# rjzhb/VectorSearch-RBAC

Hardware: AMD Instinct MI355X
Metric: QPS at recall@100, SIFT10M filtered-kNN (role RBAC), 1/2/4/8 MI355X (higher is better)
Workload: dtype int8 planes -> i32 (exact: bit-identical to the fp32 distances of vector.c)

## Files before the change

### vectorsearch-rbac_amd/csrc/vsr_device.h

```cpp
#pragma once
#include <hip/hip_runtime.h>
#include <stdint.h>
#include "vsr_bounds.h"

namespace vsr {

using f32x4 = __attribute__((ext_vector_type(4))) float;
using u32x4 = __attribute__((ext_vector_type(4))) uint32_t;
using i32x4 = __attribute__((ext_vector_type(4))) int;
using bf16x8 = __attribute__((ext_vector_type(8))) __bf16;
using f16x8 = __attribute__((ext_vector_type(8))) _Float16;

#ifdef __HIPCC__
template <class T> using gptr = const __attribute__((address_space(1))) T*;
template <class T> __device__ __forceinline__ gptr<T> as_global(const T* p) { return (gptr<T>) p; }
template <class T> __device__ __forceinline__ T lds_peek(const T* p)
{
    return *(const volatile __attribute__((address_space(3))) T*) p;
}
__device__ __forceinline__ uint2 load_tile(gptr<uint2> tiles, uint32_t t)
{
    const uint64_t v = ((gptr<uint64_t>) tiles)[t];
    return make_uint2((uint32_t) v, (uint32_t) (v >> 32));
}
// ... 16 lines not shown
    const uint64_t* bitmap;
    uint32_t        n_tiles;
    uint32_t        q_begin;
    uint32_t        q_count;
    uint32_t        block_begin;
    uint32_t        n_blocks;
    uint32_t        partial_begin;
};

struct FusedTail {
    uint32_t        enable;
    uint32_t        fan;
    ScanGroup       group;
    uint32_t*       done;
    const int64_t*  block_ids;
    const int32_t*  doc_ids;
    const int64_t*  orig_rows;
    int64_t*        out_block;
    int32_t*        out_doc;
    int64_t*        out_row;
    float*          out_dist;
    uint64_t*       out_keys;
    int32_t*        out_count;
    int32_t*        out_flag;
    int32_t*        flag_total;
    uint32_t        row_offset;
    int             metric;
    uint64_t*       dbg;
};

#ifndef VSR_MW_DENSE
#define VSR_MW_DENSE 1
#endif

struct ScanParams {
    const float4*    rows;
    const float*     norm2;
    uint32_t         n_rows;
    uint32_t         stride4;
    const float*     queries;
    const float*     q_norm2;
    const ScanGroup* groups;
    uint32_t         n_groups;
    const uint32_t*  q_slots;
    uint64_t*        partial;
    uint32_t         kp;
    uint32_t         k;
    uint32_t         cap;
    uint32_t         qmax;
    uint64_t*        cand;
    uint32_t         rw;
    const uint64_t*  tau_init;
    uint32_t         sample_stride;
    const uint2*     block_map;
    const uint4*     scr;
    const uint4*     q_scr;
    uint32_t         pstride4;
    const uint4*     scr_c;
    const uint4*     q_scr_c;
    uint32_t         cstride4;
    uint32_t         plane_ho;
    uint64_t*        qcand;
    uint32_t*        qcnt;
    uint32_t         capq;
    const uint32_t*  rank;
    const uint64_t*  ones;
    uint32_t*        err;
    uint32_t         epi;
    uint32_t         k2i;
    uint32_t         dense;
    FusedTail        fused;
    const uint64_t*  sp_off;
    const uint2*     sp_tab;
    uint32_t         sp_slots;
    const double*    sp_qtot;
};

struct SelectQuery {
    uint32_t ids_begin;
    uint32_t n_lists;
    uint32_t out_slot;
    uint32_t dst_list;
    uint32_t allowed;
    uint32_t pad;
};

constexpr uint32_t SEL_FINAL = 0xFFFFFFFFu;
constexpr uint32_t SEL_SEED = 0xFFFFFFFEu;

struct SelectParams {
    uint64_t*          tau_out;
    int32_t*           out_flags;
    int32_t*           flagged_total;
    int                seeded;
    uint64_t*          partial;
    const uint32_t*    list_ids;
    const SelectQuery* queries;
    uint32_t           kp;
    uint32_t           k;
    uint32_t           cap;
    int                metric;
    uint32_t           row_offset;
    const int64_t*     block_ids;
// ... 243 lines not shown
```

### vectorsearch-rbac_amd/csrc/vsr_mfmaw.h

```cpp
#pragma once
#include <type_traits>
#include "vsr_device.h"
#include "vsr_scan.h"
#include "vsr_topk.h"
#include "vsr_mfma.h"
#include "vsr_i8s.h"
#include "vsr_i8r.h"

namespace vsr {

constexpr int MW_THREADS = 256;
constexpr int MW_WAVES = 4;
constexpr int MW_S = 16;
constexpr int MW_ROWS = 64;
constexpr int MW_NQ = MF_NQ * MW_WAVES;
constexpr int MW_RING = 8;

#ifndef VSR_MW_DEPTH1
#define VSR_MW_DEPTH1 1
#endif
#ifndef VSR_MW_OCC1
#define VSR_MW_OCC1 3
#endif
#ifndef VSR_ABLATE
// ... 11 lines not shown
#define VSR_MW_OCC8 4
#endif
#ifndef VSR_MW_OCCL
#define VSR_MW_OCCL 2
#endif
constexpr int mw_occ(int nch, int pl = 0, bool sample = false)
{
    (void) sample;
    return pl == 2 ? VSR_MW_OCC8 : nch == 1 ? VSR_MW_OCC1 : nch == 0 ? VSR_MW_OCCL : 2;
}

__device__ __forceinline__ void lds_barrier()
{
    asm volatile("s_waitcnt lgkmcnt(0)\n\ts_barrier" ::: "memory");
}

template <int METRIC, int NCH, bool SAMPLE, int PL, int DEPTH, int EPI = 0, int NGT = 1, bool DENSE = false>
__global__ __launch_bounds__(MW_THREADS, mw_occ(NCH, PL, SAMPLE)) void mfma_wide_kernel(const ScanParams p)
{
    constexpr bool HO = PL == 1, I8 = PL == 2;
    constexpr bool LONG = NCH == 0;
    constexpr int NCHR = LONG ? 1 : NCH;
    constexpr int SR = I8 ? 8 : MW_S;
    constexpr int NU = I8 ? 2 : 4;
    static_assert(!I8 || (NCH == 1 && METRIC == M_L2), "int8 planes: one stage (d <= 128), L2 only");
    static_assert(!LONG || DEPTH == 1, "long rows: one stage ahead");
    static_assert(!DENSE || (I8 && !SAMPLE), "dense rows: the int8 main launch only");
    static_assert(DEPTH >= 1 && DEPTH <= 4 && DEPTH + 2 <= MW_RING, "row-mapping ring too short");
    extern __shared__ __align__(16) unsigned char smem[];
    const int tid = threadIdx.x;
    const int lane = tid & 63;
    const int wave = __builtin_amdgcn_readfirstlane(tid >> 6);

    uint32_t lo = 0, mapped_block = 0;
    if (p.block_map) {
        const uint2 m = p.block_map[blockIdx.x];
        if (m.x == 0xFFFFFFFFu) return;
        lo = m.x;
        mapped_block = m.y;
    } else {
        uint32_t hi = p.n_groups;
        while (hi - lo > 1) {
            const uint32_t mid = (lo + hi) >> 1;
            if (p.groups[mid].block_begin <= blockIdx.x) lo = mid; else hi = mid;
        }
    }
    const ScanGroup grp = p.groups[lo];
    const uint32_t local_block = p.block_map ? mapped_block : blockIdx.x - grp.block_begin;
    const auto g_tiles = as_global(grp.tiles);
    const auto g_bitmap = as_global(grp.bitmap);
    const auto g_norm2 = as_global(p.norm2);
    const auto g_ones = as_global(p.ones);
    const auto g_rank = as_global(p.rank);

    const uint32_t pstride4 = p.pstride4;
    const uint32_t q_count = grp.q_count;
    const bool sample_fine = SAMPLE && (grp.partial_begin & 1u);

    uint4*    stage = reinterpret_cast<uint4*>(smem);
    unsigned char* after = smem + 2 * MW_ROWS * SR * 16;
    int32_t*  rowidx = reinterpret_cast<int32_t*>(after);
    float*    rownorm = reinterpret_cast<float*>(after + MW_RING * 64 * 4);
    unsigned char* pend = after + MW_RING * 64 * 8;
    uint32_t* pend_v = reinterpret_cast<uint32_t*>(pend) + (size_t) wave * MW_PEND;
    uint32_t* pend_r = reinterpret_cast<uint32_t*>(pend + 4 * MW_PEND * 4) + (size_t) wave * MW_PEND;
    uint32_t* pend_c = reinterpret_cast<uint32_t*>(pend + 8 * MW_PEND * 4) + (size_t) wave * MW_PEND;
    constexpr bool ITEST = I8 && EPI == 1 && !SAMPLE && METRIC == M_L2;
    int32_t* rowthr = reinterpret_cast<int32_t*>(pend + 12 * MW_PEND * 4);

    const uint32_t ngt = (q_count + MF_NQ - 1) / MF_NQ;
    const uint32_t rsplit = ngt == 1 ? 4u : ngt == 2 ? 2u : 1u;
    const uint32_t g0 = (uint32_t) wave / rsplit;
    const uint32_t sub0 = ((uint32_t) wave % rsplit) * (4u / rsplit);
    const bool gact = g0 < ngt;

    const int li = lane & 15;
    const int kq = lane >> 4;
    const int jq = li;
    constexpr int NBLK = I8 ? 2 : HO ? 4 : 2;
    bf16x8 bh[NCHR][NBLK], bm[NCHR][NBLK];
    const uint4* my_qsrc = nullptr;
    i32x4 b8[NBLK];
    const uint32_t my_qi = g0 * MF_NQ + (uint32_t) jq < (uint32_t) MW_NQ ? g0 * MF_NQ + (uint32_t) jq : 0u;
    float my_qn;
    uint32_t my_slot;
    uint64_t my_tau;
    {
        const uint32_t slot = p.q_slots[grp.q_begin + (my_qi < q_count ? my_qi : 0)];
        my_slot = slot;
        my_tau = p.tau_init ? p.tau_init[slot] : KEY_EMPTY;
        my_qn = p.q_norm2[slot];
        const uint4* qsrc = p.q_scr + (size_t) slot * (HO ? 2 * pstride4 : pstride4);
        my_qsrc = qsrc;
        if constexpr (I8) {
#pragma unroll
            for (int blk = 0; blk < NBLK; ++blk) b8[blk] = __builtin_bit_cast(i32x4, qsrc[blk * 4 + kq]);
        } else {
#pragma unroll
            for (int s = 0; s < NCHR; ++s)
#pragma unroll
                for (int blk = 0; blk < NBLK; ++blk) {
                    bh[s][blk] = __builtin_bit_cast(bf16x8, qsrc[s * (HO ? 32 : 16) + blk * 4 + kq]);
                    bm[s][blk] = __builtin_bit_cast(bf16x8, qsrc[s * (HO ? 32 : 16) + (HO ? 16 : 8) + blk * 4 + kq]);
                }
        }
    }

    const uint32_t rw = p.rw, tps = MW_ROWS / rw;
    const uint32_t t0 = (uint32_t) (((uint64_t) grp.n_tiles * local_block) / grp.n_blocks);
    const uint32_t t1 = (uint32_t) (((uint64_t) grp.n_tiles * (local_block + 1)) / grp.n_blocks);
    const uint32_t n_super = (t1 - t0 + tps - 1) / tps;
    const uint32_t ss = p.sample_stride;
    const uint32_t n_it = (VSR_ABLATE & 16) ? 0u : (n_super + ss - 1) / ss;
    const bool qok = my_qi < q_count;
    const bool open = my_tau == KEY_EMPTY;
    const float tau_lim = open ? __builtin_inff() : mono_to_float((uint32_t) (my_tau >> 32));
    const int32_t c0 = !qok ? -0x40000000 : open ? 0x3FFFFFFF : (((int32_t) tau_lim - (int32_t) my_qn) + 1) >> 1;
    constexpr int NG = NGT;
    static_assert(NG == 1 || LONG, "two query groups per wave: long rows only");
    const uint32_t g1 = (uint32_t) wave + 4u;
    const bool gact2 = NG == 2 && rsplit == 1u && g1 < ngt;
    const uint32_t my_qi2 = g1 * MF_NQ + (uint32_t) jq;
    const bool qok2 = gact2 && my_qi2 < q_count;
    uint32_t my_slot2 = my_slot;
    float my_qn2 = 0.0f, tau_lim2 = -__builtin_inff();
    const uint4* my_qsrc2 = nullptr;
    bf16x8 bh2[NBLK], bm2[NBLK];
    if constexpr (NG == 2) {
        my_slot2 = p.q_slots[grp.q_begin + (qok2 ? my_qi2 : 0u)];
        const uint64_t t2 = p.tau_init ? p.tau_init[my_slot2] : KEY_EMPTY;
        tau_lim2 = t2 == KEY_EMPTY ? __builtin_inff() : mono_to_float((uint32_t) (t2 >> 32));
        my_qn2 = p.q_norm2[my_slot2];
        my_qsrc2 = p.q_scr + (size_t) my_slot2 * (HO ? 2 * pstride4 : pstride4);
#pragma unroll
        for (int blk = 0; blk < NBLK; ++blk) {
            bh2[blk] = __builtin_bit_cast(bf16x8, my_qsrc2[blk * 4 + kq]);
            bm2[blk] = __builtin_bit_cast(bf16x8, my_qsrc2[(HO ? 16 : 8) + blk * 4 + kq]);
        }
    }
    const uint32_t col_slot = lane < MF_NQ ? my_slot : my_slot2;

    const uint32_t tile_last = grp.n_tiles - 1u;
    auto fetch_desc = [&](uint32_t it_) -> uint2 {
        const uint32_t t = t0 + it_ * ss * tps + (uint32_t) lane / rw;
        const bool ok = it_ < n_it && t < t1;
        const uint2 d = load_tile(g_tiles, t < tile_last ? t : tile_last);
        return make_uint2(ok ? d.x : 0u, ok ? d.y : 0u);
    };
    int32_t  pend_row[DEPTH];
    uint64_t pend_bw[DEPTH];
    float    pend_nrm[DEPTH];
    uint2    dsc_a[DEPTH];
#pragma unroll
    for (int j = 0; j < DEPTH; ++j) {
        pend_row[j] = -1;
        pend_bw[j] = ~0ull;
        pend_nrm[j] = 0.0f;
        dsc_a[j] = make_uint2(0u, 0u);
    }
    bool bad_row = false;
    uint32_t row_lo = 0, row_hi = 0;
    if constexpr (DENSE) {
        const uint2 da = load_tile(g_tiles, t0 < tile_last ? t0 : tile_last);
        const uint2 db = load_tile(g_tiles, t1 > t0 && t1 - 1u < tile_last ? t1 - 1u : tile_last);
        row_lo = (uint32_t) __builtin_amdgcn_readfirstlane((int) da.x);
        row_hi = t1 > t0 ? (uint32_t) __builtin_amdgcn_readfirstlane((int) (db.x + db.y)) : row_lo;
        bad_row = row_hi > p.n_rows || row_hi < row_lo;
        row_hi = bad_row ? row_lo : row_hi;
    }
    auto start_dense = [&](uint32_t it_, int32_t& row, uint64_t& bw, float& nrm) {
        const uint32_t rr = row_lo + it_ * (uint32_t) MW_ROWS + (uint32_t) lane;
        const bool ok = it_ < n_it && rr < row_hi;
        row = ok ? (int32_t) rr : -1;
        bw = ~0ull;
        nrm = g_norm2[ok ? rr : 0u];
    };
    auto start_rows = [&](uint2 d, int32_t& row, uint64_t& bw, float& nrm) {
        const uint32_t r = (uint32_t) lane % rw;
        const uint32_t rr = d.x + r;
        const bool ok = r < d.y && rr < p.n_rows;
        bad_row |= r < d.y && rr >= p.n_rows;
        const uint32_t rc = ok ? rr : 0u;
        row = ok ? (int32_t) rr : -1;
        bw = *(g_bitmap ? g_bitmap + (rc >> 6) : g_ones);
        nrm = g_norm2[rc];
    };
    auto finish_rows = [&](uint32_t it_, int32_t row, uint64_t bw, float nrm) {
        if (row >= 0 && !((bw >> ((uint32_t) row & 63u)) & 1ull)) row = -1;
        if (wave == 0) {
            rowidx[(it_ % MW_RING) * 64 + lane] = row;
            rownorm[(it_ % MW_RING) * 64 + lane] = row >= 0 ? nrm : __builtin_nanf("");
            if constexpr (ITEST) rowthr[(it_ % MW_RING) * 64 + lane] = row >= 0 ? ((int32_t) nrm) >> 1 : 0x7FFFFFFF;
        }
    };
    if constexpr (DENSE) {
#pragma unroll
        for (int j = 0; j < DEPTH; ++j) {
            int32_t r0;
            uint64_t b0;
            float n0;
            start_dense((uint32_t) j, r0, b0, n0);
            finish_rows((uint32_t) j, r0, b0, n0);
            start_dense((uint32_t) (DEPTH + j), pend_row[j], pend_bw[j], pend_nrm[j]);
        }
    } else {
        uint2 d[2 * DEPTH];
#pragma unroll
        for (int j = 0; j < 2 * DEPTH; ++j) d[j] = fetch_desc((uint32_t) j);
#pragma unroll
        for (int j = 0; j < DEPTH; ++j) dsc_a[j] = fetch_desc((uint32_t) (2 * DEPTH + j));
#pragma unroll
        for (int j = 0; j < DEPTH; ++j) {
            int32_t r0;
            uint64_t b0;
            float n0;
            start_rows(d[j], r0, b0, n0);
            finish_rows((uint32_t) j, r0, b0, n0);
            start_rows(d[DEPTH + j], pend_row[j], pend_bw[j], pend_nrm[j]);
        }
    }
    __syncthreads();

    const int lrow = I8 ? tid >> 3 : tid >> 4, lchunk = I8 ? tid & 7 : tid & 15;
    constexpr int LROWS = I8 ? 32 : 16;
    uint4 X[DEPTH][NCHR][NU];
    const uint32_t last_row = p.n_rows - 1u;
    auto issue = [&](auto dc, auto sc, uint32_t it_) {
        constexpr int D = decltype(dc)::value;
        constexpr int S = decltype(sc)::value;
        const uint32_t chunk = (uint32_t) (S * SR + lchunk);
        const int32_t* ridx = rowidx + (it_ % MW_RING) * 64;
#pragma unroll
        for (int u = 0; u < NU; ++u) {
            uint32_t rc;
            if constexpr (DENSE) {
                const uint32_t rr = row_lo + it_ * (uint32_t) MW_ROWS + (uint32_t) (u * LROWS + lrow);
                rc = it_ < n_it && rr < row_hi ? rr : 0u;
            } else {
                const int32_t r = ridx[u * LROWS + lrow];
                rc = (uint32_t) (r < 0 ? 0 : r);
            }
            if ((VSR_ABLATE & 8) && it_ > 0) continue;
            const u32x4 v = *reinterpret_cast<const u32x4*>(p.scr + (size_t) (rc < last_row ? rc : last_row) * pstride4 + chunk);
            X[D][S][u] = make_uint4(v[0], v[1], v[2], v[3]);
        }
    };
    const uint32_t nch_rt = LONG ? pstride4 / (uint32_t) SR : (uint32_t) NCH;
    auto issue_rt = [&](uint32_t it_, uint32_t s_) {
        const uint32_t chunk = s_ * (uint32_t) SR + (uint32_t) lchunk;
        const int32_t* ridx = rowidx + (it_ % MW_RING) * 64;
#pragma unroll
        for (int u = 0; u < NU; ++u) {
            const int32_t r = ridx[u * LROWS + lrow];
            const uint32_t rc = (uint32_t) (r < 0 ? 0 : r);
            const u32x4 v = *reinterpret_cast<const u32x4*>(p.scr + (size_t) (rc < last_row ? rc : last_row) * pstride4 + chunk);
            X[0][0][u] = make_uint4(v[0], v[1], v[2], v[3]);
        }
    };
    auto load_b = [&](uint32_t s_, bf16x8 (&h)[NBLK], bf16x8 (&m)[NBLK]) {
#pragma unroll
        for (int blk = 0; blk < NBLK; ++blk) {
            h[blk] = __builtin_bit_cast(bf16x8, my_qsrc[s_ * (HO ? 32u : 16u) + (uint32_t) (blk * 4 + kq)]);
            m[blk] = __builtin_bit_cast(bf16x8, my_qsrc[s_ * (HO ? 32u : 16u) + (HO ? 16u : 8u) + (uint32_t) (blk * 4 + kq)]);
        }
    };
    auto issue_tile = [&](auto dc, uint32_t it_) {
        if constexpr (LONG) {
            issue_rt(it_, 0u);
            return;
        }
        issue(dc, std::integral_constant<int, 0>{}, it_);
        if constexpr (NCH > 1) issue(dc, std::integral_constant<int, 1>{}, it_);
        if constexpr (NCH > 2) issue(dc, std::integral_constant<int, 2>{}, it_);
    };
    const uint32_t n_pad = (n_it + DEPTH - 1) / DEPTH * DEPTH;
    issue_tile(std::integral_constant<int, 0>{}, 0);
    if constexpr (DEPTH > 1) issue_tile(std::integral_constant<int, 1>{}, 1);
    if constexpr (DEPTH > 2) issue_tile(std::integral_constant<int, 2>{}, 2);
    if constexpr (DEPTH > 3) issue_tile(std::integral_constant<int, 3>{}, 3);

    uint32_t p_head = 0, p_tail = 0, f_n = 0;
    constexpr int FL_R = 2;
    uint32_t f_rank[FL_R];
    uint32_t f_base = 0;
#pragma unroll
    for (int r = 0; r < FL_R; ++r) f_rank[r] = 0;
    auto flush_issue = [&]() __attribute__((always_inline)) {
        const uint32_t have = p_tail - p_head;
        f_n = have < 64u * FL_R ? have : 64u * FL_R;
        uint32_t col[FL_R];
#pragma unroll
        for (int r = 0; r < FL_R; ++r) {
            const uint32_t e = (uint32_t) (r * 64 + lane);
            col[r] = e < f_n ? pend_c[(p_head + e) % MW_PEND] : 0xFFu;
        }
        uint32_t mine = 0;
#pragma unroll
        for (int c = 0; c < MF_NQ * NG; ++c) {
            uint32_t before = 0;
#pragma unroll
            for (int r = 0; r < FL_R; ++r) {
                const uint64_t m = __ballot(col[r] == (uint32_t) c);
                if (col[r] == (uint32_t) c)
                    f_rank[r] = before + __builtin_amdgcn_mbcnt_hi((uint32_t) (m >> 32), __builtin_amdgcn_mbcnt_lo((uint32_t) m, 0u));
                before += (uint32_t) __popcll(m);
            }
            if (lane == c) mine = before;
        }
        if (lane < MF_NQ * NG && mine) f_base = atomicAdd(p.qcnt + col_slot, mine);
    };
    auto flush_store = [&]() __attribute__((always_inline)) {
#pragma unroll
        for (int r = 0; r < FL_R; ++r) {
            const uint32_t e = (uint32_t) (r * 64 + lane);
            const uint32_t idx = (p_head + e) % MW_PEND;
            const uint32_t c = e < f_n ? pend_c[idx] : 0u;
            const uint32_t base = (uint32_t) __shfl((int) f_base, (int) c);
            const uint32_t slot = (uint32_t) __shfl((int) col_slot, (int) c);
            if (e < f_n) {
                const uint32_t row = pend_r[idx];
                const uint32_t at = base + f_rank[r];
                if (at < p.capq)
                    p.qcand[(size_t) slot * p.capq + at] = ((uint64_t) pend_v[idx] << 32) | (g_rank ? g_rank[row] : row);
            }
        }
        p_head += f_n;
        f_n = 0;
    };
    auto park_mask = [&](uint64_t act, bool has, uint32_t key_hi, uint32_t row, uint32_t col = 0xFFFFFFFFu, uint32_t slot_ = 0u)
                         __attribute__((always_inline)) {
        if (col == 0xFFFFFFFFu) {
            col = (uint32_t) jq;
            slot_ = my_slot;
        }
        const uint32_t room = MW_PEND - (p_tail - p_head);
        const uint32_t rank = __builtin_amdgcn_mbcnt_hi((uint32_t) (act >> 32), __builtin_amdgcn_mbcnt_lo((uint32_t) act, 0u));
        if (has) {
            if (rank < room) {
                const uint32_t at = (p_tail + rank) % MW_PEND;
                pend_v[at] = key_hi;
                pend_r[at] = row;
                pend_c[at] = col;
            } else {
                const uint32_t ga = atomicAdd(p.qcnt + slot_, 1u);
                if (ga < p.capq) p.qcand[(size_t) slot_ * p.capq + ga] = ((uint64_t) key_hi << 32) | (g_rank ? g_rank[row] : row);
            }
        }
        const uint32_t n_act = (uint32_t) __popcll(act);
        p_tail += n_act < room ? n_act : room;
    };
    auto park = [&](bool has, uint32_t key_hi, uint32_t row, uint32_t col = 0xFFFFFFFFu, uint32_t slot_ = 0u)
                    __attribute__((always_inline)) {
        park_mask(__ballot(has), has, key_hi, row, col, slot_);
    };

    auto run = [&](auto nsc) {
// ... 378 lines not shown
```

### vectorsearch-rbac_amd/csrc/vsr_plan.h

```cpp
#pragma once
#include "vsr_runtime.h"

namespace vsr {

constexpr uint32_t SEL_FANIN = 64;

struct PlanScalars {
    uint32_t n_blocks = 0;
    int      qi = 1;
    bool     mq = false;
    bool     k2 = false;
    bool     k2w = false;
    bool     int8 = false;
    bool     class_view = false;
    bool     k2g = false;
    bool     sparse_global = false;
    uint32_t keep = 0;
    uint32_t rerank_base = 0;
    uint32_t n_scan_lists = 0;
    uint32_t qmax = 1;
    bool     k2i_sample = false;
    bool     k2r_sample = false;
    uint32_t n_blocks_s = 0;
    uint32_t n_partial_s = 0;
    uint32_t n_partial = 0;
    bool     sel_wave = false;
    uint32_t n_launch = 0;
    int64_t  scan_rows = 0;
    int64_t  scan_bytes = 0;
    float    kp_frac = 0;
    uint32_t sample_stride = 1;
    int64_t  scan_pairs = 0;
    int64_t  unique_rows = 0;
};

struct Plan : PlanScalars {
    std::vector<uint32_t>    q_slots;
    std::vector<ScanGroup>   groups;
    std::vector<uint32_t>    list_ids;
    std::vector<SelectQuery> sel1;
    std::vector<SelectQuery> selq;
    std::vector<ScanGroup>   groups_s;
    std::vector<SelectQuery> seedq;
    std::vector<uint2>       block_map;

    void reset()
    {
        static_cast<PlanScalars&>(*this) = PlanScalars{};
        q_slots.clear(); groups.clear(); list_ids.clear(); sel1.clear(); selq.clear(); groups_s.clear(); seedq.clear(); block_map.clear();
    }
};

bool make_plan(const vsr_ctx* ctx, const vsr_corpus* c, int nq, int k, int metric, bool allow_screening, bool allow_wide,
               bool allow_gemm, const vsr_filter* const* filters, Plan& plan);

inline double seed_lambda(uint32_t kp, double frac) { return (double) kp * frac; }
uint32_t seed_rank(uint32_t kp, double frac);

std::string scan_kernel_name(const Plan& plan, const vsr_corpus* c, int metric, bool k2i = false);

}
```

### vectorsearch-rbac_amd/csrc/vsr_plan.hip

```cpp
#include "vsr_plan.h"

#include <cmath>
#include <cstdio>

namespace {

struct PlanIn {
    const vsr_ctx*           ctx;
    const vsr_corpus*        c;
    int                      nq, k, metric;
    const vsr_filter* const* filters;
    const vsr_filter* filter(uint32_t q) const { return filters ? filters[q] : nullptr; }
};

struct PassItem { const vsr_filter* part; uint32_t slot; };
struct Pass {
    const vsr_filter* f; uint32_t q_off, q_count; int64_t rows; uint32_t n_tiles; int64_t cost;
    const uint2* vtiles;
};

constexpr uint32_t XCDS = 8;

struct PlanScratch {
    std::vector<PassItem> raw, items;
    std::vector<uint32_t> gid;
    std::vector<uint32_t> gend;
    std::vector<const vsr_filter*> gpart;
    std::vector<Pass>     passes;
    std::vector<uint32_t> loff, lcur, lids, lids_s, lcnt_s, level2;
    std::vector<double>   gdens_s;
    std::vector<double>   est;
    std::vector<uint2>    lane[XCDS];
};

struct Width {
    bool     mq_ok, k2_ok, k2w_ok, k2g, i8wide;
    int      wq;
    int      qmax;
    uint32_t keep, keep_c;
};

struct LaunchSize {
    int64_t  budget;
    int64_t  total_cost;
    uint32_t seed_div;
};

int64_t group_items(const PlanIn& in, PlanScratch& s)
{
    static std::atomic<uint64_t> g_epoch{0};
    const uint64_t epoch = g_epoch.fetch_add(1, std::memory_order_relaxed) + 1;
    s.raw.clear(); s.gid.clear(); s.gend.clear(); s.gpart.clear();
    const bool decompose = in.nq >= 32 && !in.ctx->no_classes;
    uint32_t null_group = 0xFFFFFFFFu;
    auto add = [&](const vsr_filter* f, uint32_t q) {
        uint32_t g;
        if (!f) {
            if (null_group == 0xFFFFFFFFu) {
                null_group = (uint32_t) s.gpart.size();
                s.gpart.push_back(nullptr);
                s.gend.push_back(0);
            }
            g = null_group;
        } else {
            if (f->plan_epoch != epoch) {
// ... 135 lines not shown
    bool any = false;
    for (const Pass& p : passes) {
        const vsr_filter* f = p.f;
        if (f && f->scanned_rows == 0) continue;
        if (!f || f->view_class < 0 || (size_t) f->view_class >= v->rows.size() || f->mode != VSR_FILTER_RANGES || f->d_bitmap ||
            f->allowed_rows != f->scanned_rows || f->scanned_rows != (int64_t) v->rows[(size_t) f->view_class])
            return false;
        any = true;
    }
    if (!any) return false;
    for (Pass& p : passes) {
        if (!p.f || p.f->scanned_rows == 0) continue;
        const size_t cls = (size_t) p.f->view_class;
        p.vtiles = v->d_tiles + v->start[cls] / 16;
        p.n_tiles = (v->rows[cls] + 15) / 16;
    }
    return true;
}

LaunchSize size_launch(const PlanIn& in, const Plan& plan, const std::vector<Pass>& passes)
{
    const vsr_ctx* ctx = in.ctx;
    int64_t total_rows = 0;
    LaunchSize ls{};
    for (auto& p : passes) {
        total_rows += std::max<int64_t>(p.rows, 1);
        ls.total_cost += p.cost;
    }
    const int64_t cus = ctx->prop.multiProcessorCount;
    ls.budget = ctx->block_budget > 0 ? ctx->block_budget : in.nq == 1 ? 2 * cus : 4 * cus;
    ls.seed_div = ctx->seed_block_div;
    if (ctx->block_budget <= 0 && plan.qi == 4) {
        const int64_t want = plan.k2g ? std::min<int64_t>(total_rows / 2048, 3 * cus)
                           : plan.k2w ? std::min<int64_t>(total_rows / 4096, 12 * cus) : std::min<int64_t>(total_rows / 13000, 16 * cus);
        if (want > ls.budget) {
            ls.budget = want;
            ls.seed_div = std::max<uint32_t>(ls.seed_div, (uint32_t) (ls.budget / (2 * cus)));
        }
    }
    if (plan.k2w) {
        const int64_t slots = (plan.k2g ? 1 : plan.int8 ? 4 : 3) * cus * ctx->sample_rounds;
        ls.seed_div = (uint32_t) std::max<int64_t>(1, (ls.budget + slots - 1) / slots);
    }
    return ls;
}

void emit_groups(const PlanIn& in, bool i8wide, const LaunchSize& ls, PlanScratch& s, Plan& plan)
{
    const vsr_ctx* ctx = in.ctx;
    const vsr_corpus* c = in.c;
    s.gdens_s.clear();
    s.loff.assign((size_t) in.nq + 1, 0);
    for (auto& p : s.passes) {
        if (p.n_tiles == 0 || p.rows == 0) continue;
        int64_t nb = (int64_t) (((__int128) p.cost * ls.budget + ls.total_cost - 1) / ls.total_cost);
        const int64_t min_rows = p.q_count > 1 ? std::max<int64_t>(ctx->min_rows_per_block, ctx->min_shared_rows) : ctx->min_rows_per_block;
        nb = std::min<int64_t>(nb, std::max<int64_t>(1, p.rows / min_rows));
        nb = std::min<int64_t>(nb, std::max<uint32_t>(1, p.n_tiles));
        nb = std::max<int64_t>(nb, 1);
        ScanGroup g;
        g.tiles = p.vtiles ? p.vtiles : p.f ? p.f->d_tiles : plan.k2w ? c->d_all_tiles : nullptr;
        g.bitmap = p.f ? p.f->d_bitmap : nullptr;
        g.n_tiles = p.n_tiles;
        g.q_begin = p.q_off;
        g.q_count = p.q_count;
        g.block_begin = plan.n_blocks;
        g.n_blocks = (uint32_t) nb;
        g.partial_begin = plan.n_partial;
        plan.groups.push_back(g);
        const double dens = p.f && p.f->scanned_rows > 0 ? (double) p.f->allowed_rows / (double) p.f->scanned_rows : 1.0;
        ScanGroup gs = g;
        gs.n_blocks = (uint32_t) std::max<int64_t>(1, nb / ls.seed_div);
        gs.block_begin = plan.n_blocks_s;
        gs.partial_begin = plan.n_partial_s;
        if (i8wide && p.q_count > 64) {
            ScanGroup g1 = gs;
            g1.q_count = (p.q_count / 2 + 15) / 16 * 16;
            plan.groups_s.push_back(g1);
            s.gdens_s.push_back(dens);
            plan.n_blocks_s += g1.n_blocks;
            plan.n_partial_s += g1.n_blocks * g1.q_count;
            gs.q_begin += g1.q_count;
            gs.q_count = p.q_count - g1.q_count;
            gs.block_begin = plan.n_blocks_s;
            gs.partial_begin = plan.n_partial_s;
            plan.n_partial_s -= gs.n_blocks * p.q_count - gs.n_blocks * gs.q_count;
        }
        plan.groups_s.push_back(gs);
        s.gdens_s.push_back(dens);
        for (uint32_t qi = 0; qi < p.q_count; ++qi) s.loff[plan.q_slots[p.q_off + qi] + 1] += g.n_blocks;
        plan.n_blocks += g.n_blocks;
        plan.n_partial += g.n_blocks * p.q_count;
        plan.n_blocks_s += gs.n_blocks;
        plan.n_partial_s += gs.n_blocks * p.q_count;
        plan.scan_rows += p.rows;
        plan.scan_pairs += p.rows * (int64_t) p.q_count;
        const int64_t row_bytes = c->bit ? (c->dim + 7) / 8 : (int64_t) c->dim * (c->half ? 2 : 4);
        const int64_t rows_bytes = c->sparse ? (int64_t) ((__int128) p.rows * (__int128) c->sp_entries * 8 / std::max<int64_t>(c->n, 1))
                                             : p.rows * row_bytes;
        plan.scan_bytes += rows_bytes + (g.bitmap ? (p.rows + 7) / 8 : 0) + (int64_t) p.q_count * in.k * 12 +
                           (plan.k2 ? p.rows * 4 : 0);
    }
    plan.n_scan_lists = plan.n_partial;
    plan.n_launch = plan.n_blocks;
}

void map_blocks_to_xcds(std::vector<uint2> (&lane)[XCDS], Plan& plan)
{
    for (auto& l : lane) l.clear();
    size_t gi = 0;
    while (gi < plan.groups.size()) {
        size_t ge = gi + 1;
        while (ge < plan.groups.size() && plan.groups[ge].tiles == plan.groups[gi].tiles &&
               plan.groups[ge].bitmap == plan.groups[gi].bitmap && plan.groups[ge].n_tiles == plan.groups[gi].n_tiles &&
               plan.groups[ge].n_blocks == plan.groups[gi].n_blocks)
            ++ge;
        for (uint32_t j = 0; j < plan.groups[gi].n_blocks; ++j) {
            uint32_t best = 0;
            for (uint32_t l = 1; l < XCDS; ++l)
                if (lane[l].size() < lane[best].size()) best = l;
            for (size_t g2 = gi; g2 < ge; ++g2) lane[best].push_back(make_uint2((uint32_t) g2, j));
        }
        gi = ge;
    }
    size_t longest = 0;
    for (auto& l : lane) longest = std::max(longest, l.size());
    plan.block_map.assign(longest * XCDS, make_uint2(0xFFFFFFFFu, 0u));
    for (uint32_t l = 0; l < XCDS; ++l)
        for (size_t t = 0; t < lane[l].size(); ++t) plan.block_map[t * XCDS + l] = lane[l][t];
    plan.n_launch = (uint32_t) plan.block_map.size();
}

double sampled_tiles(const ScanGroup& g, int rw, double tile_rows, double ss, double& t)
{
    t = std::ceil((double) g.n_tiles * rw / tile_rows);
    const double per_block = std::ceil(t / g.n_blocks);
    return std::min(t, g.n_blocks * std::ceil(per_block / ss));
}

double densest_fraction(const std::vector<ScanGroup>& groups, int rw, double tile_rows, double ss)
{
    double frac = 1.0 / ss;
    for (const ScanGroup& g : groups) {
        double t;
        const double sampled = sampled_tiles(g, rw, tile_rows, ss, t);
        if (t > 0) frac = std::max(frac, sampled / t);
    }
    return frac;
}

bool try_k2i_sample(const PlanIn& in, PlanScratch& s, Plan& plan)
{
    const vsr_corpus* c = in.c;
    const double ss = in.ctx->sample_stride;
    const double frac = densest_fraction(plan.groups_s, c->shape.rw, 32.0, ss);
    const uint32_t seed_m = seed_rank(plan.keep, frac);
    s.est.assign((size_t) in.nq, 0.0);
    for (size_t gi = 0; gi < plan.groups_s.size(); ++gi) {
        const ScanGroup& gs = plan.groups_s[gi];
        const double t32 = std::ceil((double) gs.n_tiles * c->shape.rw / 32.0);
        const double per_block = std::floor(t32 / gs.n_blocks);
        const double st = std::max(1.0, std::ceil(per_block / ss));
        const double waves = std::min(4.0, st);
// ... 154 lines not shown
        if (plan.sel_wave && sd.n_lists > 64) sd.n_lists = 64;
        plan.list_ids.insert(plan.list_ids.end(), sl, sl + sd.n_lists);
        plan.seedq[q] = sd;
    }
    if (plan.k2) {
        plan.rerank_base = plan.n_partial;
        for (size_t i = 0; i < plan.selq.size(); ++i) plan.selq[i].dst_list = plan.rerank_base + (uint32_t) i;
        plan.n_partial += (uint32_t) plan.selq.size();
    }
}

}

uint32_t vsr::seed_rank(uint32_t kp, double frac)
{
    const double lambda = seed_lambda(kp, frac);
    return (uint32_t) std::ceil(lambda + 6.0 * std::sqrt(lambda)) + 4;
}

bool vsr::make_plan(const vsr_ctx* ctx, const vsr_corpus* c, int nq, int k, int metric, bool allow_screening, bool allow_wide,
                    bool allow_gemm, const vsr_filter* const* filters, Plan& plan)
{
    static thread_local PlanScratch s;
    const PlanIn in{ctx, c, nq, k, metric, filters};
    plan.reset();
    plan.unique_rows = group_items(in, s);
    const Width w = choose_width(in, s.gend, allow_screening, allow_wide, allow_gemm);
    const uint32_t widest = cut_passes(in, w, s.items, s.passes, plan.q_slots);
    set_family(in, w, widest, plan);
    plan.class_view = take_class_view(in, plan, s.passes);
    const LaunchSize ls = size_launch(in, plan, s.passes);
    emit_groups(in, w.i8wide, ls, s, plan);
    if (plan.k2 || plan.mq) map_blocks_to_xcds(s.lane, plan);
    if (plan.k2w) {
        const bool ok = plan_wide_sampling(in, s, plan);
        plan.k2r_sample = ok && plan.class_view && plan.k2i_sample && ctx->sample_reg;
        return ok;
    }
    build_select_items(in, ls.seed_div, s, plan);
    return true;
}

std::string vsr::scan_kernel_name(const Plan& plan, const vsr_corpus* c, int metric, bool k2i)
{
    static const char* mname[] = {"L2", "IP", "COSINE", "L1", "HAMMING", "JACCARD"};
    char buf[160];
    const uint32_t nstage = (c->stride4 + 15) / 16;
    if (plan.k2g)
        snprintf(buf, sizeof buf, "vsr::gemm_screen_kernel<%s, SAMPLE=false> (K2g, bf16 coarse planes)", mname[metric]);
    else if (plan.k2w && plan.int8 && k2i)
        snprintf(buf, sizeof buf, "vsr::i8_stream_kernel<NQG=4> (K2i, int8 planes, %s)", mname[metric]);
    else if (plan.k2w && plan.int8)
        snprintf(buf, sizeof buf, "vsr::mfma_wide_kernel<%s, NCH=1, SAMPLE=false, PL=int8> (K2w, int8 planes)", mname[metric]);
    else if (plan.k2w)
        snprintf(buf, sizeof buf, "vsr::mfma_wide_kernel<%s, NCH=%u, SAMPLE=false, HO=%s> (K2w, bf16 %s planes)", mname[metric],
                 c->pstride4 / 16, c->scr_has_mid ? "false" : "true", c->scr_has_mid ? "hi+mid" : "hi-only");
    else if (plan.k2 && c->half) {
        const uint32_t hstage = (c->stride4 / 2 + 15) / 16;
        const int ng = plan.qmax > 16 ? 2 : 1;
        snprintf(buf, sizeof buf, "vsr::mfmah_scan_kernel<%s, NSTR=%u, SAMPLE=false, NG=%d> (K2h, half rows)", mname[metric],
                 hstage <= 2 ? hstage : hstage <= 4 && ng == 1 ? 4u : 0u, ng);
    } else if (plan.k2)
        snprintf(buf, sizeof buf, "vsr::mfma_scan_kernel<%s, NSTR=%d, SAMPLE=false, NG=%d> (K2)", mname[metric],
                 nstage > 4 ? 0 : 4, plan.qmax > 16 ? 2 : 1);
    else if (c->sparse)
        snprintf(buf, sizeof buf, "vsr::scans_kernel<%s, LPR=%d, QI=%d, TAB=%s> (K1s, sparse rows)", mname[metric], c->shape.lpr, plan.qi,
// ... 14 lines not shown
```

### vectorsearch-rbac_amd/csrc/vsr_search.hip

```cpp
#include "vsr_plan.h"
#include "vsr_shortlist.h"

#include <chrono>
#include <cmath>
#include <cstdio>

namespace {

using Clock = std::chrono::steady_clock;
double us_since(Clock::time_point t0) { return std::chrono::duration<double, std::micro>(Clock::now() - t0).count(); }

struct Timed {
    vsr_ctx*    ctx;
    hipStream_t stream;
    int         kind;
    hipEvent_t  a = nullptr, b = nullptr;
    hipError_t  err = hipSuccess;
    static hipEvent_t take_event(vsr_ctx* ctx)
    {
        if (!ctx->event_pool.empty()) {
            hipEvent_t e = ctx->event_pool.back();
            ctx->event_pool.pop_back();
            return e;
        }
// ... 200 lines not shown
    rr.flagged_total = ctx->d_flag_total;
    return rr;
}

void count_scan(vsr_ctx* ctx, const Plan& plan, int cls)
{
    ctx->stats.scan_bytes[cls] += plan.scan_bytes;
    ctx->stats.scan_rows[cls] += plan.scan_rows;
    ctx->stats.scan_pairs[cls] += plan.scan_pairs;
    ctx->stats.unique_rows[cls] += plan.unique_rows;
}

struct Call { const float *h_queries, *d_queries; int nq, dim, k, metric; Outputs out; const SparseQueries* sparse = nullptr; };

int search_wide(vsr_ctx* ctx, vsr_corpus* c, const Plan& plan, const Call& q)
{
    const uint32_t kp = plan.keep;
    const int nq = q.nq, metric = q.metric;
    const size_t qfloats = (size_t) c->stride4 * 4;
    const size_t q_pstride = c->scr_has_mid ? c->pstride4 : 2 * (size_t) c->pstride4;
    Staging sb;
    sb.add((size_t) nq * qfloats * sizeof(float));
    const size_t off_qn = sb.add((size_t) nq * sizeof(float));
    const size_t off_qp = sb.add((size_t) nq * q_pstride * 16);
    const size_t off_qc = sb.add(plan.k2g ? coarse_plane_u4((uint64_t) nq, c->cstride4) * 16 : 0);
    const size_t off_q8 = sb.add(plan.int8 ? (size_t) nq * 128 : 0);
    const size_t off_qn8 = sb.add(plan.int8 ? (size_t) nq * sizeof(float) : 0);
    const size_t off_qb = sb.add(plan.int8 ? (size_t) nq * sizeof(uint32_t) : 0);
    const size_t off_g = sb.add(plan.groups);
    const size_t off_gs = sb.add(plan.groups_s);
    const size_t off_qs = sb.add(plan.q_slots);
    const size_t off_sq = sb.add(plan.selq);
    const size_t off_bm = sb.add(plan.block_map);

    StageParams st{};
    RCCHK(stage_host_part(ctx, sb, off_qn, off_g, q.h_queries, q.d_queries, nq, q.dim, qfloats, st));
    RCCHK(ctx->d_cand.reserve((size_t) nq * GQ_CAP * sizeof(uint64_t)));
    RCCHK(ctx->d_samp.reserve((size_t) nq * GQ_SAMPLE_CAP * sizeof(uint64_t)));
    RCCHK(ctx->d_qcnt.reserve((size_t) 2 * nq * sizeof(uint32_t)));
    char* ds = ctx->d_desc.as<char>();

    Timed whole(ctx, 5, ctx->stream);
    uint32_t* qcnt = ctx->d_qcnt.as<uint32_t>();
    uint32_t* scnt = qcnt + nq;
    st.q_scr = reinterpret_cast<uint4*>(ds + off_qp);
    st.pstride4 = c->pstride4;
    st.plane_ho = c->scr_has_mid ? 0u : 1u;
    st.qcnt = qcnt;
    st.scnt = scnt;
    if (plan.k2g) {
        st.q_scr = nullptr;
        st.q_scr_c = reinterpret_cast<uint4*>(ds + off_qc);
        st.cstride4 = c->cstride4;
    }
    if (plan.int8) {
        RCCHK(ensure_q8_word(ctx));
        st.q_scr8 = reinterpret_cast<uint4*>(ds + off_q8);
        st.q_norm2_8 = reinterpret_cast<float*>(ds + off_qn8);
        st.q8_bad = reinterpret_cast<uint32_t*>(ds + off_qb);
        st.q8_bad_host = reinterpret_cast<uint32_t*>(ctx->h_q8.dp);
    }
    RCCHK(launch_staging(ctx, st));

    ScanParams sp = scan_params(ctx, c, kp, plan.qmax);
    sp.queries = reinterpret_cast<const float*>(ds);
    sp.q_norm2 = reinterpret_cast<const float*>(ds + off_qn);
// ... 41 lines not shown
                                                                            ctx->d_tau.as<uint64_t>(), (uint32_t) nq, ctx->stream));
        HIPCHK(sample.stop());
        hipStream_t main_stream = ctx->stream;
        if (ctx->scan_lane) {
            if (!c->scan_stream) HIPCHK(hipStreamCreateWithFlags(&c->scan_stream, hipStreamNonBlocking));
            if (!ctx->lane_in) {
                HIPCHK(hipEventCreateWithFlags(&ctx->lane_in, hipEventDisableTiming));
                HIPCHK(hipEventCreateWithFlags(&ctx->lane_out, hipEventDisableTiming));
            }
            HIPCHK(hipEventRecord(ctx->lane_in, ctx->stream));
            HIPCHK(hipStreamWaitEvent(c->scan_stream, ctx->lane_in, 0));
            main_stream = c->scan_stream;
        }
        Timed main(ctx, 1, main_stream);
        sp.groups = reinterpret_cast<const ScanGroup*>(ds + off_g);
        sp.n_groups = (uint32_t) plan.groups.size();
        sp.sample_stride = 1;
        {
            const double f = plan.kp_frac > 0 ? plan.kp_frac / kp : 1.0 / 16;
            const double admitted = kp + 6.0 * std::sqrt(kp / f) + 4.0 / f;
            const double rows_per_query = (double) plan.scan_pairs / std::max(1, nq);
            sp.epi = rows_per_query > 0 && 1024.0 * admitted / rows_per_query <= 4.0 ? 1u : 0u;
        }
        if (ctx->force_epi >= 0) sp.epi = (uint32_t) ctx->force_epi;
        if (plan.int8 && plan.qmax > 64) sp.epi = 1u;
        sp.k2i = plan.int8 && !plan.k2g && sp.epi == 1 && !ctx->no_k2i && sp.rw == 16 && sp.qmax <= 128 ? 1u : 0u;
        ctx->last_k2i = sp.k2i != 0;
        sp.dense = plan.class_view && VSR_MW_DENSE ? 1u : 0u;
        sp.tau_init = ctx->d_tau.as<uint64_t>();
        sp.qcand = ctx->d_cand.as<uint64_t>();
        sp.qcnt = qcnt;
        sp.capq = GQ_CAP;
        if (!plan.block_map.empty() && !ctx->no_xcd_map) sp.block_map = reinterpret_cast<const uint2*>(ds + off_bm);
        HIPCHK(launch_pass(sp.block_map ? plan.n_launch : plan.n_blocks, main_stream));
        HIPCHK(main.stop());
        if (ctx->scan_lane) {
            HIPCHK(hipEventRecord(ctx->lane_out, main_stream));
            HIPCHK(hipStreamWaitEvent(ctx->stream, ctx->lane_out, 0));
        }
        ctx->last_kernel = scan_kernel_name(plan, c, metric, ctx->last_k2i);
        if (plan.k2r_sample) ctx->last_kernel += " + sample vsr::i8_sample_reg_kernel<NQG=4> (K2r)";
        else if (plan.k2i_sample) ctx->last_kernel += " + sample vsr::i8_stream_kernel<NQG=4, SAMPLE=true>";
        else if (plan.int8) ctx->last_kernel += " + sample vsr::mfma_wide_kernel<L2, NCH=1, SAMPLE=true, PL=int8>";
        count_scan(ctx, plan, 1);
    }

    Timed select(ctx, 2, ctx->stream);
    RerankParams rr = rerank_params(ctx, c, ds, off_sq, kp, q.k, metric, q.out);
    rr.qcand = ctx->d_cand.as<uint64_t>();
    rr.qcnt = qcnt;
    rr.capq = GQ_CAP;
    rr.err_g = plan.k2g ? coarse_err_g(c->dim) : plane_err_g(c->dim);
    rr.err_tight = plan.k2g ? 1u : 0u;
    rr.qbad = plan.int8 ? reinterpret_cast<const uint32_t*>(ds + off_qb) : nullptr;
    rr.exact_screen = plan.int8 ? 1u : 0u;
    rr.seeded = 1;
    rr.tau_init = ctx->d_tau.as<uint64_t>();
    HIPCHK((wave_select ? launch_select_emit_wave : launch_select_rerank)(rr, (uint32_t) nq, ctx->stream));
    if (plan.n_blocks) ctx->last_kernel += wave_select ? " + select vsr::select_emit_wave_kernel" : " + select vsr::select_rerank_kernel";
    HIPCHK(select.stop());
    HIPCHK(whole.stop());
    ctx->stats.queries += nq;
    return VSR_OK;
}

uint32_t fused_fan(const vsr_ctx* ctx, const vsr_corpus* c, const Plan& plan, const Call& q)
{
// ... 697 lines not shown
```

Baseline: 3.472 million.

## Precompute per-block row-range records and issue dense row loads before query setup

For the dense class-view int8 scan, the host now precomputes a per-block record (row range, query begin, query count). The kernel reads this single record instead of doing the group binary search and the two tile loads used to derive the row bounds. This lets it issue the first row-plane loads and norm loads before loading query state, and it drops the prologue __syncthreads. Candidate rank lookups are also hoisted into flush_issue so they overlap with the prefix scan. Separately, the block budget for class-view k2w plans is halved, which means fewer, larger blocks.

```diff
diff --git a/vectorsearch-rbac_amd/csrc/vsr_device.h b/vectorsearch-rbac_amd/csrc/vsr_device.h
--- a/vectorsearch-rbac_amd/csrc/vsr_device.h
+++ b/vectorsearch-rbac_amd/csrc/vsr_device.h
@@ -72,6 +72,11 @@
 #ifndef VSR_MW_DENSE
 #define VSR_MW_DENSE 1
 #endif
+#ifndef VSR_MW_RECORD
+#define VSR_MW_RECORD 1
+#endif
+
+using BlockRecord = uint4;
 
 struct ScanParams {
     const float4*    rows;
@@ -109,6 +114,7 @@
     uint32_t         epi;
     uint32_t         k2i;
     uint32_t         dense;
+    const BlockRecord* block_rec;
     FusedTail        fused;
     const uint64_t*  sp_off;
     const uint2*     sp_tab;
diff --git a/vectorsearch-rbac_amd/csrc/vsr_mfmaw.h b/vectorsearch-rbac_amd/csrc/vsr_mfmaw.h
--- a/vectorsearch-rbac_amd/csrc/vsr_mfmaw.h
+++ b/vectorsearch-rbac_amd/csrc/vsr_mfmaw.h
@@ -67,20 +67,37 @@
     const int lane = tid & 63;
     const int wave = __builtin_amdgcn_readfirstlane(tid >> 6);
 
+    constexpr bool REC = DENSE && VSR_MW_RECORD;
     uint32_t lo = 0, mapped_block = 0;
-    if (p.block_map) {
-        const uint2 m = p.block_map[blockIdx.x];
-        if (m.x == 0xFFFFFFFFu) return;
-        lo = m.x;
-        mapped_block = m.y;
+    uint32_t row_lo = 0, row_hi = 0;
+    bool bad_row = false;
+    uint32_t n_it = 0;
+    ScanGroup grp{};
+    if constexpr (REC) {
+        const BlockRecord r = p.block_rec[blockIdx.x];
+        const uint32_t r_hi = (uint32_t) __builtin_amdgcn_readfirstlane((int) r.y);
+        grp.q_count = (uint32_t) __builtin_amdgcn_readfirstlane((int) r.w);
+        if (grp.q_count == 0u) return;
+        row_lo = (uint32_t) __builtin_amdgcn_readfirstlane((int) r.x);
+        bad_row = r_hi > p.n_rows || r_hi < row_lo;
+        row_hi = bad_row ? row_lo : r_hi;
+        grp.q_begin = (uint32_t) __builtin_amdgcn_readfirstlane((int) r.z);
+        n_it = (VSR_ABLATE & 16) ? 0u : (row_hi - row_lo + (uint32_t) MW_ROWS - 1u) / (uint32_t) MW_ROWS;
     } else {
-        uint32_t hi = p.n_groups;
-        while (hi - lo > 1) {
-            const uint32_t mid = (lo + hi) >> 1;
-            if (p.groups[mid].block_begin <= blockIdx.x) lo = mid; else hi = mid;
-        }
-    }
-    const ScanGroup grp = p.groups[lo];
+        if (p.block_map) {
+            const uint2 m = p.block_map[blockIdx.x];
+            if (m.x == 0xFFFFFFFFu) return;
+            lo = m.x;
+            mapped_block = m.y;
+        } else {
+            uint32_t hi = p.n_groups;
+            while (hi - lo > 1) {
+                const uint32_t mid = (lo + hi) >> 1;
+                if (p.groups[mid].block_begin <= blockIdx.x) lo = mid; else hi = mid;
+            }
+        }
+        grp = p.groups[lo];
+    }
     const uint32_t local_block = p.block_map ? mapped_block : blockIdx.x - grp.block_begin;
     const auto g_tiles = as_global(grp.tiles);
     const auto g_bitmap = as_global(grp.bitmap);
@@ -102,6 +119,49 @@
     uint32_t* pend_c = reinterpret_cast<uint32_t*>(pend + 8 * MW_PEND * 4) + (size_t) wave * MW_PEND;
     constexpr bool ITEST = I8 && EPI == 1 && !SAMPLE && METRIC == M_L2;
     int32_t* rowthr = reinterpret_cast<int32_t*>(pend + 12 * MW_PEND * 4);
+
+    const int lrow = I8 ? tid >> 3 : tid >> 4, lchunk = I8 ? tid & 7 : tid & 15;
+    constexpr int LROWS = I8 ? 32 : 16;
+    uint4 X[DEPTH][NCHR][NU];
+    const uint32_t last_row = p.n_rows - 1u;
+    auto issue = [&](auto dc, auto sc, uint32_t it_) {
+        constexpr int D = decltype(dc)::value;
+        constexpr int S = decltype(sc)::value;
+        const uint32_t chunk = (uint32_t) (S * SR + lchunk);
+        const int32_t* ridx = rowidx + (it_ % MW_RING) * 64;
+#pragma unroll
+        for (int u = 0; u < NU; ++u) {
+            uint32_t rc;
+            if constexpr (DENSE) {
+                const uint32_t rr = row_lo + it_ * (uint32_t) MW_ROWS + (uint32_t) (u * LROWS + lrow);
+                rc = it_ < n_it && rr < row_hi ? rr : 0u;
+            } else {
+                const int32_t r = ridx[u * LROWS + lrow];
+                rc = (uint32_t) (r < 0 ? 0 : r);
+            }
+            if ((VSR_ABLATE & 8) && it_ > 0) continue;
+            const u32x4 v = *reinterpret_cast<const u32x4*>(p.scr + (size_t) (rc < last_row ? rc : last_row) * pstride4 + chunk);
+            X[D][S][u] = make_uint4(v[0], v[1], v[2], v[3]);
+        }
+    };
+    auto start_dense = [&](uint32_t it_, int32_t& row, uint64_t& bw, float& nrm) {
+        const uint32_t rr = row_lo + it_ * (uint32_t) MW_ROWS + (uint32_t) lane;
+        const bool ok = it_ < n_it && rr < row_hi;
+        row = ok ? (int32_t) rr : -1;
+        bw = ~0ull;
+        nrm = g_norm2[ok ? rr : 0u];
+    };
+    int32_t  e_row[2 * DEPTH];
+    uint64_t e_bw[2 * DEPTH];
+    float    e_nrm[2 * DEPTH];
+    auto issue_early = [&]() __attribute__((always_inline)) {
+        issue(std::integral_constant<int, 0>{}, std::integral_constant<int, 0>{}, 0);
+        if constexpr (DEPTH > 1) issue(std::integral_constant<int, 1>{}, std::integral_constant<int, 0>{}, 1);
+        if constexpr (DEPTH > 2) issue(std::integral_constant<int, 2>{}, std::integral_constant<int, 0>{}, 2);
+        if constexpr (DEPTH > 3) issue(std::integral_constant<int, 3>{}, std::integral_constant<int, 0>{}, 3);
+#pragma unroll
+        for (int j = 0; j < 2 * DEPTH; ++j) start_dense((uint32_t) j, e_row[j], e_bw[j], e_nrm[j]);
+    };
 
     const uint32_t ngt = (q_count + MF_NQ - 1) / MF_NQ;
     const uint32_t rsplit = ngt == 1 ? 4u : ngt == 2 ? 2u : 1u;
@@ -123,6 +183,7 @@
     {
         const uint32_t slot = p.q_slots[grp.q_begin + (my_qi < q_count ? my_qi : 0)];
         my_slot = slot;
+        if constexpr (REC) issue_early();
         my_tau = p.tau_init ? p.tau_init[slot] : KEY_EMPTY;
         my_qn = p.q_norm2[slot];
         const uint4* qsrc = p.q_scr + (size_t) slot * (HO ? 2 * pstride4 : pstride4);
@@ -142,11 +203,14 @@
     }
 
     const uint32_t rw = p.rw, tps = MW_ROWS / rw;
-    const uint32_t t0 = (uint32_t) (((uint64_t) grp.n_tiles * local_block) / grp.n_blocks);
-    const uint32_t t1 = (uint32_t) (((uint64_t) grp.n_tiles * (local_block + 1)) / grp.n_blocks);
-    const uint32_t n_super = (t1 - t0 + tps - 1) / tps;
+    uint32_t t0 = 0, t1 = 0;
     const uint32_t ss = p.sample_stride;
-    const uint32_t n_it = (VSR_ABLATE & 16) ? 0u : (n_super + ss - 1) / ss;
+    if constexpr (!REC) {
+        t0 = (uint32_t) (((uint64_t) grp.n_tiles * local_block) / grp.n_blocks);
+        t1 = (uint32_t) (((uint64_t) grp.n_tiles * (local_block + 1)) / grp.n_blocks);
+        const uint32_t n_super = (t1 - t0 + tps - 1) / tps;
+        n_it = (VSR_ABLATE & 16) ? 0u : (n_super + ss - 1) / ss;
+    }
     const bool qok = my_qi < q_count;
     const bool open = my_tau == KEY_EMPTY;
     const float tau_lim = open ? __builtin_inff() : mono_to_float((uint32_t) (my_tau >> 32));
@@ -193,9 +257,7 @@
         pend_nrm[j] = 0.0f;
         dsc_a[j] = make_uint2(0u, 0u);
     }
-    bool bad_row = false;
-    uint32_t row_lo = 0, row_hi = 0;
-    if constexpr (DENSE) {
+    if constexpr (DENSE && !REC) {
         const uint2 da = load_tile(g_tiles, t0 < tile_last ? t0 : tile_last);
         const uint2 db = load_tile(g_tiles, t1 > t0 && t1 - 1u < tile_last ? t1 - 1u : tile_last);
         row_lo = (uint32_t) __builtin_amdgcn_readfirstlane((int) da.x);
@@ -203,13 +265,6 @@
         bad_row = row_hi > p.n_rows || row_hi < row_lo;
         row_hi = bad_row ? row_lo : row_hi;
     }
-    auto start_dense = [&](uint32_t it_, int32_t& row, uint64_t& bw, float& nrm) {
-        const uint32_t rr = row_lo + it_ * (uint32_t) MW_ROWS + (uint32_t) lane;
-        const bool ok = it_ < n_it && rr < row_hi;
-        row = ok ? (int32_t) rr : -1;
-        bw = ~0ull;
-        nrm = g_norm2[ok ? rr : 0u];
-    };
     auto start_rows = [&](uint2 d, int32_t& row, uint64_t& bw, float& nrm) {
         const uint32_t r = (uint32_t) lane % rw;
         const uint32_t rr = d.x + r;
@@ -228,7 +283,15 @@
             if constexpr (ITEST) rowthr[(it_ % MW_RING) * 64 + lane] = row >= 0 ? ((int32_t) nrm) >> 1 : 0x7FFFFFFF;
         }
     };
-    if constexpr (DENSE) {
+    if constexpr (REC) {
+#pragma unroll
+        for (int j = 0; j < DEPTH; ++j) {
+            finish_rows((uint32_t) j, e_row[j], e_bw[j], e_nrm[j]);
+            pend_row[j] = e_row[DEPTH + j];
+            pend_bw[j] = e_bw[DEPTH + j];
+            pend_nrm[j] = e_nrm[DEPTH + j];
+        }
+    } else if constexpr (DENSE) {
 #pragma unroll
         for (int j = 0; j < DEPTH; ++j) {
             int32_t r0;
@@ -254,32 +317,8 @@
             start_rows(d[DEPTH + j], pend_row[j], pend_bw[j], pend_nrm[j]);
         }
     }
-    __syncthreads();
-
-    const int lrow = I8 ? tid >> 3 : tid >> 4, lchunk = I8 ? tid & 7 : tid & 15;
-    constexpr int LROWS = I8 ? 32 : 16;
-    uint4 X[DEPTH][NCHR][NU];
-    const uint32_t last_row = p.n_rows - 1u;
-    auto issue = [&](auto dc, auto sc, uint32_t it_) {
-        constexpr int D = decltype(dc)::value;
-        constexpr int S = decltype(sc)::value;
-        const uint32_t chunk = (uint32_t) (S * SR + lchunk);
-        const int32_t* ridx = rowidx + (it_ % MW_RING) * 64;
-#pragma unroll
-        for (int u = 0; u < NU; ++u) {
-            uint32_t rc;
-            if constexpr (DENSE) {
-                const uint32_t rr = row_lo + it_ * (uint32_t) MW_ROWS + (uint32_t) (u * LROWS + lrow);
-                rc = it_ < n_it && rr < row_hi ? rr : 0u;
-            } else {
-                const int32_t r = ridx[u * LROWS + lrow];
-                rc = (uint32_t) (r < 0 ? 0 : r);
-            }
-            if ((VSR_ABLATE & 8) && it_ > 0) continue;
-            const u32x4 v = *reinterpret_cast<const u32x4*>(p.scr + (size_t) (rc < last_row ? rc : last_row) * pstride4 + chunk);
-            X[D][S][u] = make_uint4(v[0], v[1], v[2], v[3]);
-        }
-    };
+    if constexpr (!REC) __syncthreads();
+
     const uint32_t nch_rt = LONG ? pstride4 / (uint32_t) SR : (uint32_t) NCH;
     auto issue_rt = [&](uint32_t it_, uint32_t s_) {
         const uint32_t chunk = s_ * (uint32_t) SR + (uint32_t) lchunk;
@@ -309,10 +348,12 @@
         if constexpr (NCH > 2) issue(dc, std::integral_constant<int, 2>{}, it_);
     };
     const uint32_t n_pad = (n_it + DEPTH - 1) / DEPTH * DEPTH;
-    issue_tile(std::integral_constant<int, 0>{}, 0);
-    if constexpr (DEPTH > 1) issue_tile(std::integral_constant<int, 1>{}, 1);
-    if constexpr (DEPTH > 2) issue_tile(std::integral_constant<int, 2>{}, 2);
-    if constexpr (DEPTH > 3) issue_tile(std::integral_constant<int, 3>{}, 3);
+    if constexpr (!REC) {
+        issue_tile(std::integral_constant<int, 0>{}, 0);
+        if constexpr (DEPTH > 1) issue_tile(std::integral_constant<int, 1>{}, 1);
+        if constexpr (DEPTH > 2) issue_tile(std::integral_constant<int, 2>{}, 2);
+        if constexpr (DEPTH > 3) issue_tile(std::integral_constant<int, 3>{}, 3);
+    }
 
     uint32_t p_head = 0, p_tail = 0, f_n = 0;
     constexpr int FL_R = 2;
@@ -320,6 +361,9 @@
     uint32_t f_base = 0;
 #pragma unroll
     for (int r = 0; r < FL_R; ++r) f_rank[r] = 0;
+    uint32_t f_krow[FL_R];
+#pragma unroll
+    for (int r = 0; r < FL_R; ++r) f_krow[r] = 0;
     auto flush_issue = [&]() __attribute__((always_inline)) {
         const uint32_t have = p_tail - p_head;
         f_n = have < 64u * FL_R ? have : 64u * FL_R;
@@ -328,6 +372,10 @@
         for (int r = 0; r < FL_R; ++r) {
             const uint32_t e = (uint32_t) (r * 64 + lane);
             col[r] = e < f_n ? pend_c[(p_head + e) % MW_PEND] : 0xFFu;
+            if constexpr (REC) {
+                const uint32_t row = e < f_n ? pend_r[(p_head + e) % MW_PEND] : 0u;
+                f_krow[r] = g_rank ? g_rank[row] : row;
+            }
         }
         uint32_t mine = 0;
 #pragma unroll
@@ -353,10 +401,14 @@
             const uint32_t base = (uint32_t) __shfl((int) f_base, (int) c);
             const uint32_t slot = (uint32_t) __shfl((int) col_slot, (int) c);
             if (e < f_n) {
-                const uint32_t row = pend_r[idx];
                 const uint32_t at = base + f_rank[r];
-                if (at < p.capq)
-                    p.qcand[(size_t) slot * p.capq + at] = ((uint64_t) pend_v[idx] << 32) | (g_rank ? g_rank[row] : row);
+                if constexpr (REC) {
+                    if (at < p.capq) p.qcand[(size_t) slot * p.capq + at] = ((uint64_t) pend_v[idx] << 32) | f_krow[r];
+                } else {
+                    const uint32_t row = pend_r[idx];
+                    if (at < p.capq)
+                        p.qcand[(size_t) slot * p.capq + at] = ((uint64_t) pend_v[idx] << 32) | (g_rank ? g_rank[row] : row);
+                }
             }
         }
         p_head += f_n;
diff --git a/vectorsearch-rbac_amd/csrc/vsr_plan.h b/vectorsearch-rbac_amd/csrc/vsr_plan.h
--- a/vectorsearch-rbac_amd/csrc/vsr_plan.h
+++ b/vectorsearch-rbac_amd/csrc/vsr_plan.h
@@ -43,11 +43,12 @@
     std::vector<ScanGroup>   groups_s;
     std::vector<SelectQuery> seedq;
     std::vector<uint2>       block_map;
+    std::vector<BlockRecord> block_rec;
 
     void reset()
     {
         static_cast<PlanScalars&>(*this) = PlanScalars{};
-        q_slots.clear(); groups.clear(); list_ids.clear(); sel1.clear(); selq.clear(); groups_s.clear(); seedq.clear(); block_map.clear();
+        q_slots.clear(); groups.clear(); list_ids.clear(); sel1.clear(); selq.clear(); groups_s.clear(); seedq.clear(); block_map.clear(); block_rec.clear();
     }
 };
 
diff --git a/vectorsearch-rbac_amd/csrc/vsr_plan.hip b/vectorsearch-rbac_amd/csrc/vsr_plan.hip
--- a/vectorsearch-rbac_amd/csrc/vsr_plan.hip
+++ b/vectorsearch-rbac_amd/csrc/vsr_plan.hip
@@ -31,6 +31,7 @@
     std::vector<double>   gdens_s;
     std::vector<double>   est;
     std::vector<uint2>    lane[XCDS];
+    std::vector<uint2>    grows;
 };
 
 struct Width {
@@ -232,7 +233,8 @@
     ls.seed_div = ctx->seed_block_div;
     if (ctx->block_budget <= 0 && plan.qi == 4) {
         const int64_t want = plan.k2g ? std::min<int64_t>(total_rows / 2048, 3 * cus)
-                           : plan.k2w ? std::min<int64_t>(total_rows / 4096, 12 * cus) : std::min<int64_t>(total_rows / 13000, 16 * cus);
+                           : plan.k2w ? std::min<int64_t>(total_rows / 4096, (plan.class_view ? 6 : 12) * cus)
+                                      : std::min<int64_t>(total_rows / 13000, 16 * cus);
         if (want > ls.budget) {
             ls.budget = want;
             ls.seed_div = std::max<uint32_t>(ls.seed_div, (uint32_t) (ls.budget / (2 * cus)));
@@ -250,6 +252,7 @@
     const vsr_ctx* ctx = in.ctx;
     const vsr_corpus* c = in.c;
     s.gdens_s.clear();
+    s.grows.clear();
     s.loff.assign((size_t) in.nq + 1, 0);
     for (auto& p : s.passes) {
         if (p.n_tiles == 0 || p.rows == 0) continue;
@@ -268,6 +271,10 @@
         g.n_blocks = (uint32_t) nb;
         g.partial_begin = plan.n_partial;
         plan.groups.push_back(g);
+        if (plan.class_view) {
+            const ClassView* v = c->class_view.get();
+            s.grows.push_back(make_uint2(v->start[(size_t) p.f->view_class], v->rows[(size_t) p.f->view_class]));
+        }
         const double dens = p.f && p.f->scanned_rows > 0 ? (double) p.f->allowed_rows / (double) p.f->scanned_rows : 1.0;
         ScanGroup gs = g;
         gs.n_blocks = (uint32_t) std::max<int64_t>(1, nb / ls.seed_div);
@@ -329,6 +336,27 @@
     for (uint32_t l = 0; l < XCDS; ++l)
         for (size_t t = 0; t < lane[l].size(); ++t) plan.block_map[t * XCDS + l] = lane[l][t];
     plan.n_launch = (uint32_t) plan.block_map.size();
+}
+
+void emit_block_records(const PlanIn& in, const PlanScratch& s, Plan& plan)
+{
+    auto record = [&](uint32_t gi, uint32_t j) {
+        const ScanGroup& g = plan.groups[gi];
+        const uint64_t t0 = (uint64_t) g.n_tiles * j / g.n_blocks, t1 = (uint64_t) g.n_tiles * (j + 1) / g.n_blocks;
+        const uint32_t start = s.grows[gi].x, rows = s.grows[gi].y;
+        return make_uint4(start + (uint32_t) (16 * t0), start + (uint32_t) std::min<uint64_t>(16 * t1, rows), g.q_begin, g.q_count);
+    };
+    if (!plan.block_map.empty() && !in.ctx->no_xcd_map) {
+        plan.block_rec.resize(plan.block_map.size());
+        for (size_t i = 0; i < plan.block_map.size(); ++i) {
+            const uint2 m = plan.block_map[i];
+            plan.block_rec[i] = m.x == 0xFFFFFFFFu ? make_uint4(0u, 0u, 0u, 0u) : record(m.x, m.y);
+        }
+    } else {
+        plan.block_rec.resize(plan.n_blocks);
+        for (uint32_t gi = 0; gi < (uint32_t) plan.groups.size(); ++gi)
+            for (uint32_t j = 0; j < plan.groups[gi].n_blocks; ++j) plan.block_rec[plan.groups[gi].block_begin + j] = record(gi, j);
+    }
 }
 
 double sampled_tiles(const ScanGroup& g, int rw, double tile_rows, double ss, double& t)
@@ -549,6 +577,7 @@
     const LaunchSize ls = size_launch(in, plan, s.passes);
     emit_groups(in, w.i8wide, ls, s, plan);
     if (plan.k2 || plan.mq) map_blocks_to_xcds(s.lane, plan);
+    if (plan.class_view) emit_block_records(in, s, plan);
     if (plan.k2w) {
         const bool ok = plan_wide_sampling(in, s, plan);
         plan.k2r_sample = ok && plan.class_view && plan.k2i_sample && ctx->sample_reg;
diff --git a/vectorsearch-rbac_amd/csrc/vsr_search.hip b/vectorsearch-rbac_amd/csrc/vsr_search.hip
--- a/vectorsearch-rbac_amd/csrc/vsr_search.hip
+++ b/vectorsearch-rbac_amd/csrc/vsr_search.hip
@@ -256,6 +256,7 @@
     const size_t off_qs = sb.add(plan.q_slots);
     const size_t off_sq = sb.add(plan.selq);
     const size_t off_bm = sb.add(plan.block_map);
+    const size_t off_br = sb.add(plan.block_rec);
 
     StageParams st{};
     RCCHK(stage_host_part(ctx, sb, off_qn, off_g, q.h_queries, q.d_queries, nq, q.dim, qfloats, st));
@@ -363,7 +364,12 @@
         sp.qcnt = qcnt;
         sp.capq = GQ_CAP;
         if (!plan.block_map.empty() && !ctx->no_xcd_map) sp.block_map = reinterpret_cast<const uint2*>(ds + off_bm);
-        HIPCHK(launch_pass(sp.block_map ? plan.n_launch : plan.n_blocks, main_stream));
+        const uint32_t main_blocks = sp.block_map ? plan.n_launch : plan.n_blocks;
+        if (sp.dense) {
+            if (VSR_MW_RECORD && plan.block_rec.size() != main_blocks) return fail(VSR_ERR_INVALID, "class-view plan without block records");
+            sp.block_rec = VSR_MW_RECORD ? reinterpret_cast<const BlockRecord*>(ds + off_br) : nullptr;
+        }
+        HIPCHK(launch_pass(main_blocks, main_stream));
         HIPCHK(main.stop());
         if (ctx->scan_lane) {
             HIPCHK(hipEventRecord(ctx->lane_out, main_stream));
```

Result: faster. 3.551 million, median of 6 (+2.3%).
